# RexYing/gnn-model-explainer

Hardware: NVIDIA H100
Metric: explained-nodes/sec (100 mask-opt epochs each) (higher is better)
Workload: dtype f32

## Files before the change

### gnn-model-explainer_b200/csrc/api.cu

```cuda
#include <stdarg.h>
#include <stdio.h>
#include <stdlib.h>
#include <string.h>

#include <algorithm>
#include <cmath>
#include <iterator>
#include <memory>
#include <numeric>
#include <vector>

#include "host.cuh"

static thread_local char g_err[1024] = "";

void gx_set_error(const char* fmt, ...) {
  va_list ap;
  va_start(ap, fmt);
  vsnprintf(g_err, sizeof(g_err), fmt, ap);
  va_end(ap);
}

int check_node_list(const gx_handle* h, const char* who, const int32_t* nodes, int32_t count, int32_t n_hops, int min_hops) {
  if (n_hops < 1 || n_hops >= GX_MAX_LEVELS) { gx_set_error("%s: n_hops=%d outside [1,%d]", who, n_hops, GX_MAX_LEVELS - 1); return GX_ERR_INVALID; }
// ... 329 lines not shown
  cudaDeviceProp prop;
  GX_CUDA_CHECK(cudaGetDeviceProperties(&prop, device));
  if (prop.major != 9 || prop.minor != 0) {
    gx_set_error("gx_create: device %d is sm_%d%d; this library is built for sm_90a (H100) only", device, prop.major, prop.minor);
    return GX_ERR_CUDA;
  }
  auto h = std::make_unique<gx_handle>();
  h->device = device;
  h->num_sms = prop.multiProcessorCount;
  h->l2_bytes = prop.l2CacheSize;
  std::copy(std::begin(kNodeClasses), std::end(kNodeClasses), h->classes);
  if (const char* env = getenv("GNNX_CLASS_THREADS")) {
    int v[kNumClasses], k = 0;
    const char* p = env;
    while (*p && k < kNumClasses) { v[k++] = atoi(p); while (*p && *p != ',') ++p; if (*p == ',') ++p; }
    for (int c = 0; c < k; ++c) if (v[c] >= 32 && v[c] % 32 == 0 && (v[c] <= 256 || v[c] == 512)) h->classes[c].threads = v[c];
  }
  if (const char* env = getenv("GNNX_EXCLUSIVE_TOPK")) h->exclusive_topk = atoi(env);
  if (const char* env = getenv("GNNX_HOST_TIMING")) h->host_timing = env[0] == '1';
  if (const char* env = getenv("GNNX_FORCE_STREAM")) h->force_stream = atoi(env) != 0;
  if (const char* env = getenv("GNNX_GANG")) h->gang_override = atoi(env);
  if (const char* env = getenv("GNNX_CLUSTER_SIZE")) { const int v = atoi(env); if (v == 0 || v == 1 || v == 2 || v == 4) h->cluster_size = v; }
  if (const char* env = getenv("GNNX_CLUSTER_COST")) { const long long v = atoll(env); if (v > 0) h->cluster_cost = v; }
  if (const char* env = getenv("GNNX_IEEE_EDGE")) h->ieee_edge = atoi(env) != 0;
  if (const char* env = getenv("GNNX_NODE_GENERIC")) h->node_generic = atoi(env) != 0;
  for (int i = 0; i < kNumClasses; ++i) {
    GX_CUDA_CHECK(cudaStreamCreateWithFlags(&h->side[i], cudaStreamNonBlocking));
    GX_CUDA_CHECK(cudaEventCreate(&h->ev_join[i]));
    GX_CUDA_CHECK(cudaEventCreate(&h->ev_begin[i]));
  }
  GX_CUDA_CHECK(cudaEventCreateWithFlags(&h->ev_fork, cudaEventDisableTiming));
// ... 15 lines not shown
  if (!h) { gx_set_error("gx_set_stream: NULL handle"); return GX_ERR_INVALID; }
  h->stream = (cudaStream_t)cuda_stream;
  return GX_OK;
}

int gx_sync(gx_handle* h) {
  if (!h) { gx_set_error("gx_sync: NULL handle"); return GX_ERR_INVALID; }
  GX_CUDA_CHECK(cudaSetDevice(h->device));
  GX_CUDA_CHECK(cudaStreamSynchronize(h->stream));
  return GX_OK;
}

int64_t gx_launch_count(gx_handle* h) { return h ? h->launches : 0; }

int gx_debug_set_dump(gx_handle* h, float* dev_buf) { if (!h) return GX_ERR_INVALID; h->dbg = dev_buf; return GX_OK; }

int gx_debug_ieee_edge(gx_handle* h, int on) { if (!h) return GX_ERR_INVALID; h->ieee_edge = on != 0; return GX_OK; }

int gx_model_forward(gx_handle* h, gx_memspace space, float* pred) {
  if (!h || !pred) { gx_set_error("gx_model_forward: NULL argument"); return GX_ERR_INVALID; }
  if (!h->has_graph || !h->has_model) { gx_set_error("gx_model_forward: call gx_set_model and gx_set_graph_csr first"); return GX_ERR_INVALID; }
  if (h->g.d != h->m.d) { gx_set_error("gx_model_forward: graph feat_dim %d != model input_dim %d", h->g.d, h->m.d); return GX_ERR_INVALID; }
  GX_CUDA_CHECK(cudaSetDevice(h->device));
  const size_t np_ = (size_t)h->g.N * h->m.C;
  const size_t nh = (size_t)h->m.L * h->g.N * gx_var_row_stride(h->m.hid, h->m.emb);
  const size_t npw = h->m.att ? (size_t)h->g.N * gx_round_up(std::max(h->m.d, h->m.hid), 4) : 0;
  const size_t ne = h->head.k > 0 ? (size_t)h->g.N * (h->m.hid * (h->m.L - 1) + h->m.emb) : 0;
  GX_CUDA_CHECK(h->d_fwd.reserve((nh + np_ + npw + ne) * 4));
  float* H = h->d_fwd.as<float>();
  float* pd = space == GX_DEVICE ? pred : H + nh;
// ... 339 lines not shown
```

### gnn-model-explainer_b200/csrc/explain_common.cuh

```cuda
#pragma once
#include "gnnx_internal.cuh"

namespace {

#ifndef GX_SHORT_DEPTH
#define GX_SHORT_DEPTH 1
#endif
constexpr int kLongRow = 32;

__device__ __forceinline__ float warp_sum(float x) {
#pragma unroll
  for (int o = 16; o > 0; o >>= 1) x += __shfl_xor_sync(0xffffffffu, x, o);
  return x;
}
__device__ __forceinline__ float warp_max(float x) {
#pragma unroll
  for (int o = 16; o > 0; o >>= 1) x = fmaxf(x, __shfl_xor_sync(0xffffffffu, x, o));
  return x;
}
__device__ __forceinline__ float sigmoid_f(float x) { return 1.0f / (1.0f + expf(-x)); }
__device__ __forceinline__ float sigmoid_fast(float x, bool ieee) {
  return ieee ? 1.0f / (1.0f + expf(-x)) : __fdividef(1.0f, 1.0f + __expf(-x));
}
__device__ __forceinline__ float adam_delta_fast(float m, float v, float step, float bc2s, float bc2s_inv, float eps, bool ieee) {
// ... 260 lines not shown
```

### gnn-model-explainer_b200/csrc/explain_node.cu

```cuda
#include "explain_common.cuh"

namespace {

template <typename IdxT, int HID, int EMB, bool kWpShared, bool kTrace>
__device__ __forceinline__ void readout_phase(int lane, int C, int gt, const IdxT* irp, const IdxT* icol, const float* a,
                                              const float* Yh1, const float* Yh2, float* zs, const float* bs, const float* W3s,
                                              const float* Wpp, const float* bpp, float* logit, float* dE, float* dZ3,
                                              float* tr, float* trp) {
  constexpr int HS = HID, H4 = HID / 4, PD = 2 * HID + EMB;
  const int g = lane >> 3, q8 = lane & 7;
  float4 acc = make_float4(0.f, 0.f, 0.f, 0.f);
  {
    const int r0 = irp[0], r1 = irp[1];
    if (q8 < H4) acc = gather_row<IdxT, true, 4>(r0 + g, r1, 4, icol, a, Yh2, HS, q8);
  }
#pragma unroll
  for (int o = 8; o <= 16; o <<= 1) {
    acc.x += __shfl_xor_sync(0xffffffffu, acc.x, o); acc.y += __shfl_xor_sync(0xffffffffu, acc.y, o);
    acc.z += __shfl_xor_sync(0xffffffffu, acc.z, o); acc.w += __shfl_xor_sync(0xffffffffu, acc.w, o);
  }
  if (lane < H4) st4(zs + 4 * lane, acc);
  __syncwarp();
  const int le = lane < EMB ? lane : EMB - 1;
  const int lh = lane < HID ? lane : HID - 1;
// ... 110 lines not shown
    if (tid == 0 && crank == 0) peer.sti(&s_task, atomicAdd(A.counter, 1));
    phase_sync<CS>();
    const int qi = s_task;
    phase_sync<CS>();
    if (qi >= A.ntasks) break;
    const int task_id = A.order[qi];
    if (A.dbg != nullptr && tid == 0) {
      unsigned long long t_start_ns;
      asm volatile("mov.u64 %0, %%globaltimer;" : "=l"(t_start_ns));
      s_clk[7] = (long long)t_start_ns;
    }
    const GxTask* __restrict__ Tp = A.plan.tasks + task_id;
    const int n = Tp->n, n1 = Tp->n1, n2 = Tp->n2, e1 = Tp->e1, np = Tp->npairs_in;
    const int gt = hp.mode ? __ldg(A.g.pred_label + Tp->node) : Tp->gt_label;
    const int64_t node_off = Tp->node_off, rp_off = Tp->rp_off, edge_off = Tp->edge_off, pair_off = Tp->pair_off;
    if (tid == 0) sL = gx_make_layout(n, n1, n2, e1, d, HID, EMB, C, nwarps, (int)sizeof(IdxT), CS);
    __syncthreads();
    const int dp = sL.dp, D4 = dp / 4;
    const int32_t* __restrict__ lo2gid = A.plan.lo2gid + node_off;

    {
      float* const X = base + sL.X; float* const W1s = base + sL.W1s; float* const W2s = base + sL.W2s; float* const W3s = base + sL.W3s;
      float* const bs = base + sL.bs; float* const sF = base + sL.sF; float* const Fm = base + sL.F; float* const mF = base + sL.mF;
      float* const vF = base + sL.vF; float* const gFp = base + sL.gFp; float* const a = base + sL.a; float* const yv = base + sL.y;
      float2* const MM = reinterpret_cast<float2*>(A.pws + (int64_t)cid * A.pws_stride_words); float2* const mm = MM + np; float2* const vv = mm + np; float2* const SS = vv + np;
      uint2* const PX = reinterpret_cast<uint2*>(SS + np);
      IdxT* const icol = reinterpret_cast<IdxT*>(base + sL.icol); IdxT* const irp = reinterpret_cast<IdxT*>(base + sL.irp);
    for (int idx = tid; idx < n * dp; idx += nthreads) {
      const int i = idx / dp, f = idx - i * dp;
      X[idx] = f < d ? __ldg(A.g.feat + (int64_t)lo2gid[i] * d + f) : 0.f;
    }
    for (int idx = tid; idx < dp * HS; idx += nthreads) {
      const int f = idx / HS, c = idx - f * HS;
      W1s[idx] = f < d ? __ldg(m.W[0] + f * HID + c) : 0.f;
    }
    for (int idx = tid; idx < HID * HS; idx += nthreads) W2s[idx] = __ldg(m.W[1] + idx);
    {
      float* const W1t = base + sL.W1t; float* const W2t = base + sL.W2t;
      for (int idx = tid; idx < HID * dp; idx += nthreads) {
// ... 18 lines not shown
      sF[f] = hp.mode ? 1.0f : 0.5f;
      Fm[f] = 0.f; mF[f] = 0.f; vF[f] = 0.f;
      if (resume && A.x.feat_state_in != nullptr && f < d) {
        const float* fs = A.x.feat_state_in + (int64_t)task_id * 3 * d;
        Fm[f] = fs[f]; mF[f] = fs[d + f]; vF[f] = fs[2 * d + f];
        sF[f] = sigmoid_f(fs[f]);
      }
      if (hp.out_iter == 0 && !hp.mode && f < d) {
        if (A.out_feat != nullptr) A.out_feat[(int64_t)task_id * d + f] = sF[f];
        if (A.x.feat_state_out != nullptr) {
          float* fo = A.x.feat_state_out + (int64_t)task_id * 3 * d;
          fo[f] = Fm[f]; fo[d + f] = mF[f]; fo[2 * d + f] = vF[f];
        }
      }
    }
    for (int idx = tid; idx < cnwarps * dp; idx += nthreads) gFp[idx] = 0.f;
    const float m0_std = sqrtf(2.0f / (float)n);
    for (int p = tid; p < np; p += nthreads) {
      const int i = A.plan.pair_i[pair_off + p], j = A.plan.pair_j[pair_off + p];
      const int pij = A.plan.pair_pij[pair_off + p], pji = A.plan.pair_pji[pair_off + p];
      const int oij = A.plan.pair_oij[pair_off + p], oji = A.plan.pair_oji[pair_off + p];
      float Mi, Mj;
      if (hp.mode) {
        Mi = Mj = 0.f;
      } else if (hp.init == GX_INIT_PHILOX) {
        Mi = 1.0f + m0_std * philox_normal(hp.seed, (uint32_t)Tp->node, (uint32_t)oij);
        Mj = 1.0f + m0_std * philox_normal(hp.seed, (uint32_t)Tp->node, (uint32_t)oji);
      } else {
        Mi = __ldg(A.m0 + edge_off + oij);
        Mj = __ldg(A.m0 + edge_off + oji);
      }
// ... 204 lines not shown
            st4(dZ2 + j * HS + 4 * q, group_dense(zs + G.gbase * 4, H4, W2t, HS, q, make_float4(0.f, 0.f, 0.f, 0.f)));
          __syncwarp();
        }
      }
      __syncthreads();
      GX_MARK(3)
      {
        const IdxT* const irp = reinterpret_cast<const IdxT*>(base + sL.irp);
        const IdxT* const icol = reinterpret_cast<const IdxT*>(base + sL.icol);
        const float* const a = base + sL.a; const float* const dZ2 = base + sL.dZ2; const float* const dE = base + sL.dE;
        const float* const Yh1 = base + sL.Yh1; const float* const q1 = base + sL.q1; const float* const W1t = base + sL.W1t;
        const float* const U = base + sL.U; const float* const sF = base + sL.sF;
        const IdxT* const cnt1 = reinterpret_cast<const IdxT*>(base + sL.cnt1);
        const IdxT* const llistB = reinterpret_cast<const IdxT*>(base + sL.llistB);
        float* const dZ1s = base + sL.U;
        float* const gFp = base + sL.gFp; float* const zs = base + sL.zs + warp * 128;
        float4 gacc = make_float4(0.f, 0.f, 0.f, 0.f);
        const int ntask = nlongB1 + (n2 + epi - 1) / epi;
        for (int t = cwarp; t < ntask; t += cnwarps) {
          float4 dh;
          const int i = row_task_gather<IdxT, false, (NT >= 512 ? 1 : GX_SHORT_DEPTH)>(t, nlongB1, llistB, n2, G, H4, irp, icol, a, dZ2, HS, cnt1, zs, dh);
          const bool act = i >= 0;
          float4 yh = make_float4(0.f, 0.f, 0.f, 0.f), dy = yh;
          if (act && q < H4) {
            yh = ld4(Yh1 + i * HS + 4 * q);
            if (i == 0) { const float4 e4 = ld4(dE + 4 * q); dh.x += e4.x; dh.y += e4.y; dh.z += e4.z; dh.w += e4.w; }
            dy.x = yh.x > 0.f ? dh.x : 0.f; dy.y = yh.y > 0.f ? dh.y : 0.f;
            dy.z = yh.z > 0.f ? dh.z : 0.f; dy.w = yh.w > 0.f ? dh.w : 0.f;
          }
          const float sdot = group_sum<kGW>(yh.x * dy.x + yh.y * dy.y + yh.z * dy.z + yh.w * dy.w, G);
          if (act && q < H4) {
            const float rq = q1[i];
            st4(zs + lane * 4, make_float4((dy.x - yh.x * sdot) * rq, (dy.y - yh.y * sdot) * rq,
                                           (dy.z - yh.z * sdot) * rq, (dy.w - yh.w * sdot) * rq));
          }
          __syncwarp();
          if (act && q < D4) {
            const float4 o = group_dense(zs + G.gbase * 4, H4, W1t, dp, q, make_float4(0.f, 0.f, 0.f, 0.f));
            const float4 u = ld4(U + i * dp + 4 * q);
            const float4 s4 = ld4(sF + 4 * q);
            gacc.x = fmaf(o.x, u.x, gacc.x); gacc.y = fmaf(o.y, u.y, gacc.y);
            gacc.z = fmaf(o.z, u.z, gacc.z); gacc.w = fmaf(o.w, u.w, gacc.w);
            peer.st4(dZ1s + i * dp + 4 * q, make_float4(o.x * s4.x, o.y * s4.y, o.z * s4.z, o.w * s4.w));
          }
          __syncwarp();
        }
        st4(zs + lane * 4, gacc);
        __syncwarp();
        if (G.grp == 0 && q < D4) {
          float4 tsum = gacc;
          for (int g2 = 1; g2 < epi; ++g2) {
            const float4 o = ld4(zs + (g2 * G.GW + q) * 4);
            tsum.x += o.x; tsum.y += o.y; tsum.z += o.z; tsum.w += o.w;
          }
          peer.st4(gFp + cwarp * dp + 4 * q, tsum);
        }
        __syncwarp();
      }
      phase_sync<CS>();
      GX_MARK(4)
      if (A.dbg != nullptr && it == 1 && qi == 0 && crank == 0) {
        if (tid == 0) {
          A.dbg[0] = (float)sL.total_words; A.dbg[1] = (float)sL.X; A.dbg[2] = (float)sL.U; A.dbg[3] = (float)sL.Yh1;
          A.dbg[4] = (float)sL.q1; A.dbg[5] = (float)sL.Yh2; A.dbg[6] = (float)sL.q2; A.dbg[7] = (float)sL.dZ2;
          A.dbg[8] = (float)sL.U; A.dbg[9] = (float)sL.gFp; A.dbg[10] = (float)sL.dE; A.dbg[11] = (float)sL.dZ3;
          A.dbg[12] = (float)sL.logit; A.dbg[13] = (float)sL.a; A.dbg[14] = (float)dp; A.dbg[15] = (float)nwarps;
        }
        for (int w = tid; w < sL.total_words; w += nthreads) A.dbg[16 + w] = base[w];
      }
      {
        float* const gFp = base + sL.gFp;
        float* const sF = base + sL.sF;
        float* const Fm = base + sL.F; float* const mF = base + sL.mF; float* const vF = base + sL.vF;
        const float* const yv = base + sL.y;
        const float* const dZ1s = base + sL.U;
        float* const X = base + sL.X;
        float* const dZ2 = base + sL.dZ2;
        float* const Yh1 = base + sL.Yh1;
        float* const dZ3 = base + sL.dZ3;
        float* const Yh2 = base + sL.Yh2;
        float2* const MM = reinterpret_cast<float2*>(A.pws + (int64_t)cid * A.pws_stride_words); float2* const mm = MM + np; float2* const vv = mm + np; float2* const SS = vv + np;
        const uint2* const PX = reinterpret_cast<const uint2*>(SS + np);
        float* const a = base + sL.a;
        const int p0 = cwarp * 32 + lane, pstride = nthreads * CS;
        uint2 pxn = p0 < np ? PX[p0] : make_uint2(0u, 0u);
        const float2 tab = __ldg(hp.adam_tab + (it - 1));
        const float step = tab.x, bc2s = tab.y, bc2s_inv = 1.0f / tab.y;
        const bool last = (it == hp.out_iter);
        const float nn = (float)n * (float)n;
        const float ent_over_nn = hp.c_ent / nn;
        const float lap_over_nn = hp.c_lap / nn;
        const int fthreads = min(nthreads, gx_round_up(d, 32));
        for (int f = tid - (nthreads - fthreads); f >= 0 && f < d && !hp.mode; f += fthreads) {
          float gsum = 0.f;
          for (int w = 0; w < cnwarps; ++w) gsum += gFp[w * dp + f];
          const float s = sF[f];
          const float g = s * (1.f - s) * (gsum + hp.c_feat_size / (float)d);
          float mf = mF[f], vf = vF[f], Fv = Fm[f];
          mf = mf + (g - mf) * hp.one_minus_b1;
          vf = vf * hp.b2 + hp.one_minus_b2 * g * g;
          Fv = Fv - step * (mf / (sqrtf(vf) / bc2s + hp.eps));
          mF[f] = mf; vF[f] = vf; Fm[f] = Fv;
          const float sn = sigmoid_f(Fv);
          sF[f] = sn;
          if (last && crank == 0) {
            if (A.out_feat != nullptr) A.out_feat[(int64_t)task_id * d + f] = sn;
            if (A.x.feat_state_out != nullptr) {
              float* fo = A.x.feat_state_out + (int64_t)task_id * 3 * d;
              fo[f] = Fv; fo[d + f] = mf; fo[2 * d + f] = vf;
            }
// ... 201 lines not shown
template <typename IdxT, int HID, int EMB, int NT, int CS, bool kNarrow = false>
cudaError_t launch_one(const GxExplainLaunch& cfg, const ExplainArgs& args, cudaStream_t s) {
  if (args.x.trace != nullptr) return launch_one_t<IdxT, HID, EMB, NT, true, CS, kNarrow>(cfg, args, s);
  return launch_one_t<IdxT, HID, EMB, NT, false, CS, kNarrow>(cfg, args, s);
}

template <int HID, int EMB>
cudaError_t launch_dims(const GxExplainLaunch& cfg, const ExplainArgs& args, cudaStream_t s) {
  if (cfg.smem_bytes <= 0) return cudaErrorInvalidValue;
  if (cfg.cluster == 4) return launch_one<uint16_t, HID, EMB, 512, 4>(cfg, args, s);
  if (cfg.cluster == 2) return launch_one<uint16_t, HID, EMB, 512, 2>(cfg, args, s);
  if (cfg.cluster != 1) return cudaErrorInvalidValue;
  const bool narrow = HID == EMB && 4 * ((args.m.d + 3) / 4) <= HID && (args.hp.flags & GX_HP_NODE_GENERIC) == 0;
  if (cfg.threads <= 256)
    return narrow ? launch_one<uint16_t, HID, EMB, 256, 1, true>(cfg, args, s) : launch_one<uint16_t, HID, EMB, 256, 1>(cfg, args, s);
  return narrow ? launch_one<uint16_t, HID, EMB, 512, 1, true>(cfg, args, s) : launch_one<uint16_t, HID, EMB, 512, 1>(cfg, args, s);
}

}

int gx_explain_max_smem() { return 227 * 1024; }

cudaError_t gx_launch_outer_pairs(const GxHparamsDev& hp, const GxGraphDev& g, const GxPlanArrays& plan, int count,
                                  const float* m0, float* out_mask, const GxExtra& x, cudaStream_t s) {
  const int grid = count < GX_GRID_CAP ? count : GX_GRID_CAP;
  if (x.trace != nullptr) {
    const size_t smem = (size_t)(hp.iters > 0 ? hp.iters : 1) * 4 * sizeof(double);
    if (smem > 48 * 1024) return cudaErrorInvalidValue;
    outer_pairs_kernel<true><<<grid, 256, smem, s>>>(hp, g, plan, count, m0, out_mask, x);
  } else {
    const int slices = std::max(1, std::min(32, GX_GRID_CAP / grid));
    outer_pairs_kernel<false><<<dim3(grid, slices), 256, 0, s>>>(hp, g, plan, count, m0, out_mask, x);
  }
  return cudaGetLastError();
}

// ... 9 lines not shown
```

### gnn-model-explainer_b200/csrc/gnnx_internal.cuh

```cuda
#pragma once
#include <cuda_runtime.h>
#include <stdint.h>

#include "gnnx.h"

#define GX_MAX_LEVELS 8
#define GX_NONE16 0xFFFFu
#define GX_MAX_LAYERS 7
#define GX_MAX_GANG 160
#define GX_GRID_CAP (132 * 8)
#define GX_WP_SMEM_MAX 2048

struct GxTask {
  int32_t node;
  int32_t n;
  int32_t e_d;
  int32_t npairs;
  int32_t npairs_in;
  int32_t idx_new;
  int32_t gt_label;
  int32_t n1, n2;
  int32_t e1;
  int32_t status;
  int32_t n_norm;
// ... 82 lines not shown

#define GX_HP_IEEE_EDGE 1
#define GX_HP_NODE_GENERIC 2

struct GxExtra {
  float* trace;
  float* trace_pred;
  double* tr_outer;
  int32_t epochs;
  const float* adam_m_in; const float* adam_v_in; const float* feat_state_in;
  float* mask_param_out; float* adam_m_out; float* adam_v_out; float* feat_state_out;
};

__host__ __device__ inline int gx_round_up(int x, int m) { return (x + m - 1) / m * m; }

struct GxLayout {
  int X, U, Yh1, q1, Yh2, q2, dZ2, a, y, W1s, W1t, W2s, W2t, W3s, bs, sF, F, mF, vF, gFp, zs, dE, dZ3, logit, Wp;
  int icol, irp, llist, cnt1, llistB;
  int total_words;
  int dp;
};

__host__ __device__ inline GxLayout gx_make_layout(int n, int n1, int n2, int e1, int d,
                                                   int hid, int emb, int C, int nwarps,
                                                   int idx_bytes, int cs = 1) {
  GxLayout L;
  const int dp = gx_round_up(d, 4);
  L.dp = dp;
  int o = 0;
  auto takef = [&](int words) { int r = o; o += gx_round_up(words, 4); return r; };
  auto takei = [&](int elems) { int r = o; o += gx_round_up((elems * idx_bytes + 3) / 4, 4); return r; };
  L.X = takef(n * dp);
  L.U = takef(n2 * dp);
  L.Yh1 = takef(n2 * hid);
  L.q1 = takef(n2);
  L.Yh2 = takef(n1 * hid);
  L.q2 = takef(n1);
  L.dZ2 = takef(n1 * hid);
  L.a = takef(e1);
  L.y = takef(n);
  L.W1s = takef(dp * hid);
  L.W1t = takef(hid * dp);
  L.W2s = takef(hid * hid);
  L.W2t = takef(hid * hid);
  L.W3s = takef(hid * emb);
  L.bs = takef(2 * hid + emb);
  L.sF = takef(dp);
  L.F = takef(dp);
  L.mF = takef(dp);
  L.vF = takef(dp);
  L.gFp = takef(nwarps * cs * dp);
  L.zs = takef(nwarps * 128);
  L.dE = takef(2 * hid);
  L.dZ3 = takef(hid);
  L.logit = takef(C < 32 ? 32 : C);
  L.Wp = takef(C * (2 * hid + emb + 1) <= GX_WP_SMEM_MAX ? C * (2 * hid + emb + 1) : 0);
  L.icol = takei(e1);
  L.irp = takei(n2 + 1);
  L.llist = takei(n2);
  L.cnt1 = takei(n2);
  L.llistB = takei(n2);
  L.total_words = o;
  return L;
}

struct GxStreamLayout {
// ... 168 lines not shown
  int32_t grid;
  int32_t cluster = 1;
  int32_t gang = 1;
  unsigned long long* gang_bars = nullptr;
  int32_t* gang_mail = nullptr;
  float* gws;
  int64_t gws_stride_words;
  float* pws;
  int64_t pws_stride_words;
  float* dbg;
  GxExtra x;
};
cudaError_t gx_launch_explain(const GxExplainLaunch& cfg, const GxGraphDev& g, const GxModelDev& m,
                              const GxHparamsDev& hp, const GxPlanArrays& plan, const float* m0,
                              float* out_mask, float* out_feat, cudaStream_t s);
cudaError_t gx_launch_explain_stream(const GxExplainLaunch& cfg, const GxGraphDev& g, const GxModelDev& m,
                                     const GxHparamsDev& hp, const GxPlanArrays& plan, const float* m0,
                                     float* out_mask, float* out_feat, cudaStream_t s);
cudaError_t gx_launch_explain_gang(const GxExplainLaunch& cfg, const GxGraphDev& g, const GxModelDev& m,
                                   const GxHparamsDev& hp, const GxPlanArrays& plan, const float* m0,
                                   float* out_mask, float* out_feat, cudaStream_t s);
int gx_gang_smem_bytes(int d, int hid, int C);
cudaError_t gx_launch_model_forward(const GxGraphDev& g, const GxModelDev& m, const GxHeadDev& hd, float* H, float* pred, float* emb_out, float* P,
                                    cudaStream_t s);
constexpr int GX_STREAM_THREADS = 768;
int gx_explain_max_smem();
struct GxGraphBatchDev {
  int32_t num_graphs, max_nodes, d;
  const int32_t* rowptr;
  const int32_t* col;
// ... 53 lines not shown
```

### gnn-model-explainer_b200/csrc/host.cuh

```cuda
#pragma once
#include <stdio.h>

#include <algorithm>
#include <chrono>
#include <vector>

#include "gnnx_internal.cuh"

struct DevBuf {
  void* p = nullptr;
  size_t cap = 0;
  DevBuf() = default;
  DevBuf(const DevBuf&) = delete;
  DevBuf& operator=(const DevBuf&) = delete;
  DevBuf(DevBuf&& o) noexcept : p(o.p), cap(o.cap) { o.p = nullptr; o.cap = 0; }
  DevBuf& operator=(DevBuf&& o) noexcept { std::swap(p, o.p); std::swap(cap, o.cap); return *this; }
  ~DevBuf() { if (p) cudaFree(p); }
  cudaError_t reserve(size_t bytes) {
    if (bytes <= cap) return cudaSuccess;
    if (p) cudaFree(p);
    p = nullptr;
    cap = 0;
    size_t want = bytes + bytes / 4 + 256;
    cudaError_t e = cudaMalloc(&p, want);
    if (e == cudaSuccess) cap = want;
    return e;
  }
  template <typename T> T* as() const { return reinterpret_cast<T*>(p); }
};

struct LaunchClass {
  int cap_bytes;
  int threads;
  int ctas_per_sm;
};
constexpr LaunchClass kNodeClasses[] = {
    {13 * 1024, 128, 16}, {27 * 1024, 256, 8}, {55 * 1024, 256, 4},
    {112 * 1024, 512, 2}, {226 * 1024, 512, 1}, {0, 512, 1}, {226 * 1024, 512, 1}};
constexpr int kNumClasses = sizeof(kNodeClasses) / sizeof(kNodeClasses[0]);
constexpr int kStreamClass = 5;
constexpr int kClusterClass = 6;
constexpr int kOneClass = 4, kTwoClass = 3;

inline double now_us() { return std::chrono::duration<double, std::micro>(std::chrono::steady_clock::now().time_since_epoch()).count(); }

struct AdamKey { float lr, b1, b2, decay_rate; int32_t opt, sched, decay_step, restart, iters, start; };

struct gx_handle {
  int device = 0;
  int num_sms = 132;
  int64_t l2_bytes = (int64_t)50 << 20;
  cudaStream_t stream = nullptr;
  cudaStream_t side[kNumClasses] = {};
  cudaEvent_t ev_fork = nullptr;
  cudaEvent_t ev_t0 = nullptr, ev_t1 = nullptr;
  bool timed = false;
  float* dbg = nullptr;
  LaunchClass classes[kNumClasses];
  int exclusive_topk = 30;
  bool host_timing = false;
  bool ieee_edge = false;
  bool node_generic = false;
  int gang_override = 0;
  int cluster_size = 1;
  int64_t cluster_cost = 0;
  int plan_cluster = 1;
  bool force_stream = false;
  cudaEvent_t ev_join[kNumClasses] = {}, ev_begin[kNumClasses] = {};
  bool class_used[kNumClasses] = {};
  int64_t launches = 0;

  bool has_graph = false;
  GxGraphDev g{};
  DevBuf g_rowptr, g_col, g_feat, g_label, g_pred;
// ... 151 lines not shown
```

### gnn-model-explainer_b200/csrc/node_mode.cu

```cuda
#include <string.h>

#include <algorithm>
#include <vector>

#include "host.cuh"

namespace {

int ensure_slot_ws(gx_handle* h) {
  const int64_t N = h->g.N;
  const int W = (int)((N + 31) / 32);
  int slots = h->num_sms * 8;
  const size_t per_slot = (size_t)W * 4 + (size_t)(W + 1) * 4 + (size_t)N + (size_t)(N + 1) * 4 * 2 + (size_t)N * 4 * 2 + 64;
  const size_t budget = (size_t)4 << 30;
  while (slots > 1 && per_slot * slots > budget) slots /= 2;
  if (h->ws.slots == slots && h->ws.W == W && h->ws_buf.p) return GX_OK;
  auto al = [](size_t x) { return (x + 15) / 16 * 16; };
  size_t o = 0;
  const size_t o_bm = o; o += al((size_t)slots * W * 4);
  const size_t o_wp = o; o += al((size_t)slots * (W + 1) * 4);
  const size_t o_q = o; o += al((size_t)slots * (N + 1) * 4);
  const size_t o_loc = o; o += al((size_t)slots * N * 4);
  const size_t o_cof = o; o += al((size_t)slots * N * 4);
  const size_t o_pb = o; o += al((size_t)slots * (N + 1) * 4);
// ... 5 lines not shown
  h->ws.q = (int32_t*)(b + o_q);
  h->ws.loc = (int32_t*)(b + o_loc);
  h->ws.cof = (int32_t*)(b + o_cof);
  h->ws.pbase = (int32_t*)(b + o_pb);
  h->ws.dist = (uint8_t*)(b + o_dist);
  h->ws.W = W;
  h->ws.slots = slots;
  GX_CUDA_CHECK(cudaMemsetAsync(h->ws.bm, 0, (size_t)slots * W * 4, h->stream));
  return GX_OK;
}

int task_smem_class(const gx_handle* h, const GxTask& T, int* bytes_out) {
  const GxModelDev& m = h->m;
  const bool small_idx = !h->force_stream && T.n < 65535 && T.e1 < 65535;
  for (int c = 0; small_idx && c < kStreamClass; ++c) {
    const int nwarps = h->classes[c].threads / 32;
    const GxLayout L = gx_make_layout(T.n, T.n1, T.n2, T.e1, m.d, m.hid, m.emb, m.C, nwarps, 2);
    const int64_t bytes = (int64_t)L.total_words * 4;
    if (bytes <= h->classes[c].cap_bytes) {
      *bytes_out = (int)bytes;
      return c;
    }
  }
  *bytes_out = 0;
  return kStreamClass;
}

enum class NodeKernel { smem, cluster, gang, stream1, variant };

}

// ... 115 lines not shown
  h->plan.pair_pji = pb + 3 * tp; h->plan.pair_oij = pb + 4 * tp; h->plan.pair_oji = pb + 5 * tp;
  const double t2 = h->host_timing ? now_us() : 0.0;
  GX_CUDA_CHECK(gx_launch_khop_fill(h->g, count, n_hops, h->ws, h->plan, h->stream));
  h->launches += 1;
  const LaunchClass& cluster_cls = h->classes[kClusterClass];
  for (int c = 0; c < kNumClasses; ++c) h->class_order[c].clear();
  auto cost = [&](int32_t t) { const GxTask& T = h->tasks[t]; return (int64_t)T.e1 * (h->m.d + 2 * h->m.hid) + (int64_t)T.n2 * 600 + (int64_t)T.npairs * 60; };
  const int g_cluster_size = h->cluster_size > 1 ? h->cluster_size : 1;
  const int64_t g_cluster_cost = h->cluster_cost;
  h->plan_cluster = g_cluster_size;
  for (int t = 0; t < count; ++t) {
    GxTask& T = h->tasks[t];
    int bytes = 0;
    int cls = h->m.variant ? kStreamClass : task_smem_class(h, T, &bytes);
    if (cls < kStreamClass && g_cluster_size > 1 && cost(t) > g_cluster_cost) {
      const GxLayout L = gx_make_layout(T.n, T.n1, T.n2, T.e1, h->m.d, h->m.hid, h->m.emb, h->m.C, cluster_cls.threads / 32, 2, g_cluster_size);
      if ((int64_t)L.total_words * 4 <= cluster_cls.cap_bytes) { cls = kClusterClass; bytes = L.total_words * 4; }
    }
    T.smem_bytes = bytes;
    h->class_order[cls].push_back(t);
  }
  if (h->cluster_size == 0 && !h->m.variant && !h->force_stream && h->class_order[kStreamClass].empty()) {
    double demand = 0;
    for (int c = 0; c < kStreamClass; ++c) demand += (double)h->class_order[c].size() / h->classes[c].ctas_per_sm;
    const int spare = h->num_sms - (int)(demand + 0.999);
    std::vector<int32_t> cand;
    for (int c : {kTwoClass, kOneClass}) for (int32_t t : h->class_order[c]) cand.push_back(t);
    std::stable_sort(cand.begin(), cand.end(), [&](int32_t x, int32_t y) { return cost(x) > cost(y); });
    auto lat = [&](int32_t t) { return 6e-6 * (double)cost(t); };
    int best_cs = 1, best_k = 0;
    if (!cand.empty() && spare >= 2) {
      double best = lat(cand[0]);
      for (int cs : {2, 4}) {
        const double ovh = cs == 2 ? 0.55 : 0.8;
        int k = 0;
        while (k < (int)cand.size() && (k + 1) * cs <= spare && lat(cand[k]) / cs + ovh < lat(cand[k])) {
          const GxTask& T = h->tasks[cand[k]];
          const GxLayout L = gx_make_layout(T.n, T.n1, T.n2, T.e1, h->m.d, h->m.hid, h->m.emb, h->m.C, cluster_cls.threads / 32, 2, cs);
          if ((int64_t)L.total_words * 4 > cluster_cls.cap_bytes) break;
          ++k;
        }
        if (k == 0) continue;
        const double span = std::max(lat(cand[0]) / cs + ovh, k < (int)cand.size() ? lat(cand[k]) : 0.0);
        if (span < best * 0.95) { best = span; best_cs = cs; best_k = k; }
      }
    }
    if (best_cs > 1) {
      h->plan_cluster = best_cs;
      for (int i = 0; i < best_k; ++i) {
        const int32_t t = cand[i];
        GxTask& T = h->tasks[t];
        const GxLayout L = gx_make_layout(T.n, T.n1, T.n2, T.e1, h->m.d, h->m.hid, h->m.emb, h->m.C, cluster_cls.threads / 32, 2, best_cs);
        T.smem_bytes = L.total_words * 4;
        for (int c : {kTwoClass, kOneClass}) {
          auto& v = h->class_order[c];
          v.erase(std::remove(v.begin(), v.end(), t), v.end());
        }
        h->class_order[kClusterClass].push_back(t);
      }
    }
  }
  std::vector<int32_t> order_all;
  for (int c = 0; c < kNumClasses; ++c) {
    auto& v = h->class_order[c];
    std::stable_sort(v.begin(), v.end(), [&](int32_t x, int32_t y) { return cost(x) > cost(y); });
  }
  {
// ... 91 lines not shown
      const LaunchClass& K = h->classes[c];
      const int nt = (int)h->class_order[c].size();
      int need = 0;
      for (int32_t t : h->class_order[c]) need = std::max(need, h->tasks[t].smem_bytes);
      cfg[c].threads = K.threads;
      cfg[c].dbg = h->dbg;
      cfg[c].x = D.x;
      if (c == kClusterClass) {
        kernel[c] = NodeKernel::cluster;
        cfg[c].cluster = h->plan_cluster;
        cfg[c].grid = std::min<int>(nt, h->num_sms / h->plan_cluster) * h->plan_cluster;
        cfg[c].smem_bytes = std::max(need, K.cap_bytes - 2048);
        slabs[c] = cfg[c].grid / h->plan_cluster;
      } else if (K.cap_bytes > 0) {
        kernel[c] = NodeKernel::smem;
        cfg[c].grid = std::min<int>(nt, h->num_sms * K.ctas_per_sm);
        cfg[c].smem_bytes = c == kOneClass ? std::max(need, K.cap_bytes - 2048) : std::max(need, 1024);
        slabs[c] = cfg[c].grid;
      } else if (nt > 0) {
        int max_slabs = h->num_sms, gang = 0;
        if (!h->m.variant && h->gang_override >= 0 && h->m.d <= 128 && gx_gang_smem_bytes(h->m.d, h->m.hid, h->m.C) <= gx_explain_max_smem()) {
          int64_t ws = 1;
          for (int32_t t : h->class_order[c]) ws = std::max<int64_t>(ws, (int64_t)h->tasks[t].e_d * 8 + (int64_t)h->tasks[t].n * 240);
          const int64_t l2_budget = h->l2_bytes * 5 / 8;
          int ngangs = (int)std::max<int64_t>(1, std::min<int64_t>(std::min(nt, h->num_sms), l2_budget / ws));
          gang = std::max(1, std::min(h->num_sms / ngangs, GX_MAX_GANG));
          if (h->gang_override > 0) gang = std::min(std::min(h->gang_override, h->num_sms), GX_MAX_GANG);
          max_slabs = std::max(1, std::min(ngangs, h->num_sms / gang));
        }
        kernel[c] = h->m.variant ? NodeKernel::variant : gang > 0 ? NodeKernel::gang : NodeKernel::stream1;
// ... 74 lines not shown
```

### gnn-model-explainer_b200/gnnx/_abi.py

```python
import ctypes as C
import os

_HERE = os.path.dirname(os.path.abspath(__file__))
LIB_PATH = os.environ.get("GNNX_LIB_PATH") or os.path.join(_HERE, "lib", "libgnnx.so")

GX_OK = 0
GX_ERR_UNSUPPORTED = -3
GX_HOST, GX_DEVICE = 0, 1
GX_INIT_M0, GX_INIT_PHILOX, GX_INIT_STATE = 0, 1, 2
GX_VERSION = 211
GX_TRACE_COLS = 8
TR_LOSS_EDGES, TR_PRED, TR_SIZE, TR_ENT, TR_LAP, TR_FEAT, TR_DENSITY, TR_PGT = range(8)
GX_MODEL_BN = 1
GX_MODEL_ATT = 2
GX_MAX_HEAD_LAYERS = 4

EXPORTS = [
    "gx_default_hparams", "gx_last_error", "gx_version", "gx_create", "gx_destroy", "gx_set_stream",
    "gx_sync", "gx_set_model", "gx_set_graph_csr", "gx_neighborhood_rows", "gx_plan_nodes",
    "gx_plan_fetch", "gx_explain_nodes", "gx_densify", "gx_launch_count", "gx_last_explain_ms",
    "gx_set_graph_batch_csr", "gx_plan_graphs", "gx_explain_graphs", "gx_grad_nodes", "gx_grad_graphs",
    "gx_explain_nodes_ex", "gx_explain_graphs_ex", "gx_offedge_regularisers", "gx_offedge_regularisers_graphs",
    "gx_debug_force_stream", "gx_debug_ieee_edge", "gx_debug_set_dump", "gx_debug_set_gang", "gx_debug_set_cluster", "gx_denoise_topk",
    "gx_model_forward", "gx_comm_unique_id", "gx_comm_init", "gx_comm_destroy", "gx_count_nodes", "gx_allgather_masks", "gx_unshard_masks",
    "gx_plan_class_counts", "gx_last_class_ms", "gx_explain_nodes_unconstrained", "gx_explain_graphs_unconstrained",
    "gx_set_model_att", "gx_set_model_head", "gx_count_graphs", "gx_densify_graphs", "gx_denoise_topk_edges",
]


class GxModelDims(C.Structure):
    _fields_ = [("input_dim", C.c_int32), ("hidden_dim", C.c_int32), ("embed_dim", C.c_int32),
                ("num_classes", C.c_int32), ("num_layers", C.c_int32), ("flags", C.c_int32)]


class GxHparams(C.Structure):
    _fields_ = [("num_epochs", C.c_int32), ("lr", C.c_float), ("beta1", C.c_float), ("beta2", C.c_float),
                ("eps", C.c_float), ("coef_size", C.c_float), ("coef_feat_size", C.c_float),
                ("coef_ent", C.c_float), ("coef_lap", C.c_float), ("mask_act", C.c_int32),
# ... 61 lines not shown
    L.gx_grad_nodes.argtypes = [vp, C.c_int, f32p]
    L.gx_grad_graphs.argtypes = [vp, C.c_int, i32p, f32p]
    L.gx_denoise_topk.argtypes = [vp, C.c_int, f32p, C.c_int32, C.c_int32, f32p, i32p, i32p, f32p]
    L.gx_denoise_topk_edges.argtypes = [vp, C.c_int, f32p, C.c_int32, C.c_int32, f32p, i32p, i32p, f32p]
    L.gx_comm_unique_id.argtypes = [C.c_char_p]
    L.gx_comm_init.argtypes = [vp, C.c_int32, C.c_int32, C.c_char_p]
    L.gx_comm_destroy.argtypes = [vp]
    L.gx_count_nodes.argtypes = [vp, i32p, C.c_int32, C.c_int32, i32p, i32p]
    L.gx_allgather_masks.argtypes = [vp, f32p, C.c_int64, C.c_int64, f32p]
    L.gx_unshard_masks.argtypes = [vp, f32p, C.c_int32, i64p, i64p, i32p, f32p]
    L.gx_count_graphs.argtypes = [vp, i32p, C.c_int32, i32p, i32p]
    L.gx_densify_graphs.argtypes = [vp, C.c_int, i32p, C.c_int32, f32p, vp]
    L.gx_debug_force_stream.argtypes = [vp, C.c_int]
    L.gx_debug_ieee_edge.argtypes = [vp, C.c_int]
    L.gx_debug_set_dump.argtypes = [vp, vp]
    L.gx_model_forward.argtypes = [vp, C.c_int, f32p]
    L.gx_debug_set_gang.argtypes = [vp, C.c_int]
    L.gx_debug_set_cluster.argtypes = [vp, C.c_int, C.c_int64]
    L.gx_launch_count.argtypes = [vp]
    L.gx_plan_class_counts.argtypes = [vp, i32p, i32p, i32p]
    L.gx_last_class_ms.argtypes = [vp, f32p, f32p]
    L.gx_launch_count.restype = C.c_int64
    L.gx_last_explain_ms.argtypes = [vp, C.POINTER(C.c_float)]
    for name in EXPORTS:
        getattr(L, name)
    if L.gx_version() != GX_VERSION:
        raise ImportError("libgnnx.so is version %d, this binding expects %d -- rebuild (python __graft_entry__.py)" % (L.gx_version(), GX_VERSION))
    _lib = L
    return L

# ... 5 lines not shown
```

### include/gnnx.h

```cpp
#ifndef GNNX_H_
#define GNNX_H_

#include <stdint.h>

#ifdef __cplusplus
extern "C" {
#endif

#define GX_VERSION 211

typedef struct gx_handle gx_handle;

typedef enum gx_status {
  GX_OK = 0,
  GX_ERR_INVALID = -1,
  GX_ERR_CUDA = -2,
  GX_ERR_UNSUPPORTED = -3,
  GX_ERR_NODE = -4,
  GX_ERR_NOMEM = -5
} gx_status;

typedef enum gx_memspace { GX_HOST = 0, GX_DEVICE = 1 } gx_memspace;

typedef struct gx_model_dims {
// ... 139 lines not shown
int gx_count_graphs(gx_handle* h, const int32_t* graph_ids, int32_t count, int32_t* n_out, int32_t* e_out);
int gx_densify_graphs(gx_handle* h, gx_memspace space, const int32_t* graph_ids, int32_t count, const float* values, double* out);

int gx_model_forward(gx_handle* h, gx_memspace space, float* pred);

int64_t gx_launch_count(gx_handle* h);
int gx_plan_class_counts(gx_handle* h, int32_t counts[7], int32_t smem_bytes[7], int32_t* cluster_size);
int gx_last_class_ms(gx_handle* h, float begin_ms[7], float end_ms[7]);
int gx_last_explain_ms(gx_handle* h, float* ms);

int gx_debug_set_gang(gx_handle* h, int ctas_per_task);
int gx_debug_set_cluster(gx_handle* h, int cluster_size, int64_t min_cost);
int gx_debug_force_stream(gx_handle* h, int on);
int gx_debug_ieee_edge(gx_handle* h, int on);
int gx_debug_set_dump(gx_handle* h, float* dev_buf);

#ifdef __cplusplus
}
#endif
#endif
```

Measured before the change: 212,500.

## Store per-task feature-grad partials and compute CTA residency from occupancy API

Replaces the per-warp feature-gradient accumulator (sized by warps times cluster size) with a per-task partial buffer sized by a task-count bound. The final reduction now sums over tasks instead of over warps, which removes the zero-initialisation pass and makes the layout independent of warp count. CTAs-per-SM for each launch class is now queried from the CUDA occupancy API rather than hardcoded, and the defaults for the small classes drop from 16/8 to 8/4. The change also adds an optional 1024-thread variant and lowers the exclusive top-k default. Risks include larger shared memory for tasks with many B1 rows, and lower residency if the occupancy query is conservative.

```diff
diff --git a/gnn-model-explainer_b200/csrc/api.cu b/gnn-model-explainer_b200/csrc/api.cu
--- a/gnn-model-explainer_b200/csrc/api.cu
+++ b/gnn-model-explainer_b200/csrc/api.cu
@@ -367,7 +367,14 @@
     int v[kNumClasses], k = 0;
     const char* p = env;
     while (*p && k < kNumClasses) { v[k++] = atoi(p); while (*p && *p != ',') ++p; if (*p == ',') ++p; }
-    for (int c = 0; c < k; ++c) if (v[c] >= 32 && v[c] % 32 == 0 && (v[c] <= 256 || v[c] == 512)) h->classes[c].threads = v[c];
+    for (int c = 0; c < k; ++c)
+      if (v[c] >= 32 && v[c] % 32 == 0 && (v[c] <= 256 || v[c] == 512 || (v[c] == 1024 && c != kClusterClass))) h->classes[c].threads = v[c];
+  }
+  for (int c = 0; c < kNumClasses; ++c) {
+    if (h->classes[c].cap_bytes == 0) continue;
+    const int n = gx_node_ctas_per_sm(h->classes[c].threads, h->classes[c].cap_bytes);
+    if (n < 1) { gx_set_error("gx_create: launch class %d (%d threads, %d bytes) fits no SM", c, h->classes[c].threads, h->classes[c].cap_bytes); return GX_ERR_CUDA; }
+    h->classes[c].ctas_per_sm = n;
   }
   if (const char* env = getenv("GNNX_EXCLUSIVE_TOPK")) h->exclusive_topk = atoi(env);
   if (const char* env = getenv("GNNX_HOST_TIMING")) h->host_timing = env[0] == '1';
@@ -413,6 +420,15 @@
 int64_t gx_launch_count(gx_handle* h) { return h ? h->launches : 0; }
 
 int gx_debug_set_dump(gx_handle* h, float* dev_buf) { if (!h) return GX_ERR_INVALID; h->dbg = dev_buf; return GX_OK; }
+
+int gx_debug_class_residency(gx_handle* h, int32_t threads[7], int32_t ctas_per_sm[7]) {
+  if (!h) return GX_ERR_INVALID;
+  for (int c = 0; c < kNumClasses; ++c) {
+    if (threads) threads[c] = h->classes[c].threads;
+    if (ctas_per_sm) ctas_per_sm[c] = h->classes[c].ctas_per_sm;
+  }
+  return GX_OK;
+}
 
 int gx_debug_ieee_edge(gx_handle* h, int on) { if (!h) return GX_ERR_INVALID; h->ieee_edge = on != 0; return GX_OK; }
 
diff --git a/gnn-model-explainer_b200/csrc/explain_common.cuh b/gnn-model-explainer_b200/csrc/explain_common.cuh
--- a/gnn-model-explainer_b200/csrc/explain_common.cuh
+++ b/gnn-model-explainer_b200/csrc/explain_common.cuh
@@ -6,7 +6,6 @@
 #ifndef GX_SHORT_DEPTH
 #define GX_SHORT_DEPTH 1
 #endif
-constexpr int kLongRow = 32;
 
 __device__ __forceinline__ float warp_sum(float x) {
 #pragma unroll
diff --git a/gnn-model-explainer_b200/csrc/explain_node.cu b/gnn-model-explainer_b200/csrc/explain_node.cu
--- a/gnn-model-explainer_b200/csrc/explain_node.cu
+++ b/gnn-model-explainer_b200/csrc/explain_node.cu
@@ -148,7 +148,7 @@
     const int n = Tp->n, n1 = Tp->n1, n2 = Tp->n2, e1 = Tp->e1, np = Tp->npairs_in;
     const int gt = hp.mode ? __ldg(A.g.pred_label + Tp->node) : Tp->gt_label;
     const int64_t node_off = Tp->node_off, rp_off = Tp->rp_off, edge_off = Tp->edge_off, pair_off = Tp->pair_off;
-    if (tid == 0) sL = gx_make_layout(n, n1, n2, e1, d, HID, EMB, C, nwarps, (int)sizeof(IdxT), CS);
+    if (tid == 0) sL = gx_make_layout(n, n1, n2, e1, d, HID, EMB, C, nwarps, (int)sizeof(IdxT));
     __syncthreads();
     const int dp = sL.dp, D4 = dp / 4;
     const int32_t* __restrict__ lo2gid = A.plan.lo2gid + node_off;
@@ -156,7 +156,7 @@
     {
       float* const X = base + sL.X; float* const W1s = base + sL.W1s; float* const W2s = base + sL.W2s; float* const W3s = base + sL.W3s;
       float* const bs = base + sL.bs; float* const sF = base + sL.sF; float* const Fm = base + sL.F; float* const mF = base + sL.mF;
-      float* const vF = base + sL.vF; float* const gFp = base + sL.gFp; float* const a = base + sL.a; float* const yv = base + sL.y;
+      float* const vF = base + sL.vF; float* const a = base + sL.a; float* const yv = base + sL.y;
       float2* const MM = reinterpret_cast<float2*>(A.pws + (int64_t)cid * A.pws_stride_words); float2* const mm = MM + np; float2* const vv = mm + np; float2* const SS = vv + np;
       uint2* const PX = reinterpret_cast<uint2*>(SS + np);
       IdxT* const icol = reinterpret_cast<IdxT*>(base + sL.icol); IdxT* const irp = reinterpret_cast<IdxT*>(base + sL.irp);
@@ -205,7 +205,6 @@
         }
       }
     }
-    for (int idx = tid; idx < cnwarps * dp; idx += nthreads) gFp[idx] = 0.f;
     const float m0_std = sqrtf(2.0f / (float)n);
     for (int p = tid; p < np; p += nthreads) {
       const int i = A.plan.pair_i[pair_off + p], j = A.plan.pair_j[pair_off + p];
@@ -440,8 +439,7 @@
         const IdxT* const cnt1 = reinterpret_cast<const IdxT*>(base + sL.cnt1);
         const IdxT* const llistB = reinterpret_cast<const IdxT*>(base + sL.llistB);
         float* const dZ1s = base + sL.U;
-        float* const gFp = base + sL.gFp; float* const zs = base + sL.zs + warp * 128;
-        float4 gacc = make_float4(0.f, 0.f, 0.f, 0.f);
+        float* const gFt = base + sL.gFt; float* const zs = base + sL.zs + warp * 128;
         const int ntask = nlongB1 + (n2 + epi - 1) / epi;
         for (int t = cwarp; t < ntask; t += cnwarps) {
           float4 dh;
@@ -461,27 +459,26 @@
                                            (dy.z - yh.z * sdot) * rq, (dy.w - yh.w * sdot) * rq));
           }
           __syncwarp();
+          float4 ou = make_float4(0.f, 0.f, 0.f, 0.f);
           if (act && q < D4) {
             const float4 o = group_dense(zs + G.gbase * 4, H4, W1t, dp, q, make_float4(0.f, 0.f, 0.f, 0.f));
             const float4 u = ld4(U + i * dp + 4 * q);
             const float4 s4 = ld4(sF + 4 * q);
-            gacc.x = fmaf(o.x, u.x, gacc.x); gacc.y = fmaf(o.y, u.y, gacc.y);
-            gacc.z = fmaf(o.z, u.z, gacc.z); gacc.w = fmaf(o.w, u.w, gacc.w);
+            ou = make_float4(o.x * u.x, o.y * u.y, o.z * u.z, o.w * u.w);
             peer.st4(dZ1s + i * dp + 4 * q, make_float4(o.x * s4.x, o.y * s4.y, o.z * s4.z, o.w * s4.w));
           }
           __syncwarp();
-        }
-        st4(zs + lane * 4, gacc);
-        __syncwarp();
-        if (G.grp == 0 && q < D4) {
-          float4 tsum = gacc;
-          for (int g2 = 1; g2 < epi; ++g2) {
-            const float4 o = ld4(zs + (g2 * G.GW + q) * 4);
-            tsum.x += o.x; tsum.y += o.y; tsum.z += o.z; tsum.w += o.w;
-          }
-          peer.st4(gFp + cwarp * dp + 4 * q, tsum);
-        }
-        __syncwarp();
+          st4(zs + lane * 4, ou);
+          __syncwarp();
+          if (G.grp == 0 && q < D4) {
+            for (int g2 = 1; g2 < epi; ++g2) {
+              const float4 o = ld4(zs + (g2 * G.GW + q) * 4);
+              ou.x += o.x; ou.y += o.y; ou.z += o.z; ou.w += o.w;
+            }
+            peer.st4(gFt + t * dp + 4 * q, ou);
+          }
+          __syncwarp();
+        }
       }
       phase_sync<CS>();
       GX_MARK(4)
@@ -489,13 +486,14 @@
         if (tid == 0) {
           A.dbg[0] = (float)sL.total_words; A.dbg[1] = (float)sL.X; A.dbg[2] = (float)sL.U; A.dbg[3] = (float)sL.Yh1;
           A.dbg[4] = (float)sL.q1; A.dbg[5] = (float)sL.Yh2; A.dbg[6] = (float)sL.q2; A.dbg[7] = (float)sL.dZ2;
-          A.dbg[8] = (float)sL.U; A.dbg[9] = (float)sL.gFp; A.dbg[10] = (float)sL.dE; A.dbg[11] = (float)sL.dZ3;
-          A.dbg[12] = (float)sL.logit; A.dbg[13] = (float)sL.a; A.dbg[14] = (float)dp; A.dbg[15] = (float)nwarps;
+          A.dbg[8] = (float)sL.U; A.dbg[9] = (float)sL.gFt; A.dbg[10] = (float)sL.dE; A.dbg[11] = (float)sL.dZ3;
+          A.dbg[12] = (float)sL.logit; A.dbg[13] = (float)sL.a; A.dbg[14] = (float)dp; A.dbg[15] = (float)(nlongB1 + (n2 + epi - 1) / epi);
         }
         for (int w = tid; w < sL.total_words; w += nthreads) A.dbg[16 + w] = base[w];
       }
       {
-        float* const gFp = base + sL.gFp;
+        const float* const gFt = base + sL.gFt;
+        const int ntaskB1 = nlongB1 + (n2 + epi - 1) / epi;
         float* const sF = base + sL.sF;
         float* const Fm = base + sL.F; float* const mF = base + sL.mF; float* const vF = base + sL.vF;
         const float* const yv = base + sL.y;
@@ -519,7 +517,8 @@
         const int fthreads = min(nthreads, gx_round_up(d, 32));
         for (int f = tid - (nthreads - fthreads); f >= 0 && f < d && !hp.mode; f += fthreads) {
           float gsum = 0.f;
-          for (int w = 0; w < cnwarps; ++w) gsum += gFp[w * dp + f];
+#pragma unroll 4
+          for (int t = 0; t < ntaskB1; ++t) gsum += gFt[t * dp + f];
           const float s = sF[f];
           const float g = s * (1.f - s) * (gsum + hp.c_feat_size / (float)d);
           float mf = mF[f], vf = vF[f], Fv = Fm[f];
@@ -751,12 +750,33 @@
   const bool narrow = HID == EMB && 4 * ((args.m.d + 3) / 4) <= HID && (args.hp.flags & GX_HP_NODE_GENERIC) == 0;
   if (cfg.threads <= 256)
     return narrow ? launch_one<uint16_t, HID, EMB, 256, 1, true>(cfg, args, s) : launch_one<uint16_t, HID, EMB, 256, 1>(cfg, args, s);
-  return narrow ? launch_one<uint16_t, HID, EMB, 512, 1, true>(cfg, args, s) : launch_one<uint16_t, HID, EMB, 512, 1>(cfg, args, s);
+  if (cfg.threads <= 512)
+    return narrow ? launch_one<uint16_t, HID, EMB, 512, 1, true>(cfg, args, s) : launch_one<uint16_t, HID, EMB, 512, 1>(cfg, args, s);
+  if (cfg.threads != 1024 || args.x.trace != nullptr) return cudaErrorInvalidValue;
+  return narrow ? launch_one_t<uint16_t, HID, EMB, 1024, false, 1, true>(cfg, args, s) : launch_one_t<uint16_t, HID, EMB, 1024, false, 1, false>(cfg, args, s);
+}
+
+template <int NT>
+int ctas_per_sm(int threads, int smem_bytes) {
+  auto kern = explain_node_kernel<uint16_t, 20, 20, NT, false, 1, true>;
+  int n = 0;
+  if (cudaFuncSetAttribute(kern, cudaFuncAttributeMaxDynamicSharedMemorySize, smem_bytes) != cudaSuccess ||
+      cudaFuncSetAttribute(kern, cudaFuncAttributePreferredSharedMemoryCarveout, cudaSharedmemCarveoutMaxShared) != cudaSuccess ||
+      cudaOccupancyMaxActiveBlocksPerMultiprocessor(&n, kern, threads, (size_t)smem_bytes) != cudaSuccess)
+    return 0;
+  return n;
 }
 
 }
 
 int gx_explain_max_smem() { return 227 * 1024; }
+
+int gx_node_ctas_per_sm(int threads, int smem_bytes) {
+  if (threads < 32 || threads % 32 != 0) return 0;
+  if (threads <= 256) return ctas_per_sm<256>(threads, smem_bytes);
+  if (threads <= 512) return ctas_per_sm<512>(threads, smem_bytes);
+  return threads == 1024 ? ctas_per_sm<1024>(threads, smem_bytes) : 0;
+}
 
 cudaError_t gx_launch_outer_pairs(const GxHparamsDev& hp, const GxGraphDev& g, const GxPlanArrays& plan, int count,
                                   const float* m0, float* out_mask, const GxExtra& x, cudaStream_t s) {
diff --git a/gnn-model-explainer_b200/csrc/gnnx_internal.cuh b/gnn-model-explainer_b200/csrc/gnnx_internal.cuh
--- a/gnn-model-explainer_b200/csrc/gnnx_internal.cuh
+++ b/gnn-model-explainer_b200/csrc/gnnx_internal.cuh
@@ -120,8 +120,19 @@
 
 __host__ __device__ inline int gx_round_up(int x, int m) { return (x + m - 1) / m * m; }
 
+constexpr int kLongRow = 32;
+
+__host__ __device__ inline int gx_b1_task_bound(int n1, int n2, int e1, int d, int hid, int emb) {
+  int gw = (d + 3) / 4;
+  gw = gw > hid / 4 ? gw : hid / 4;
+  gw = gw > emb / 4 ? gw : emb / 4;
+  const int epi = gw <= 32 ? 32 / gw : 1;
+  const int nlong = n1 > kLongRow ? (n2 < e1 / (kLongRow + 1) ? n2 : e1 / (kLongRow + 1)) : 0;
+  return (n2 + epi - 1) / epi + nlong;
+}
+
 struct GxLayout {
-  int X, U, Yh1, q1, Yh2, q2, dZ2, a, y, W1s, W1t, W2s, W2t, W3s, bs, sF, F, mF, vF, gFp, zs, dE, dZ3, logit, Wp;
+  int X, U, Yh1, q1, Yh2, q2, dZ2, a, y, W1s, W1t, W2s, W2t, W3s, bs, sF, F, mF, vF, gFt, zs, dE, dZ3, logit, Wp;
   int icol, irp, llist, cnt1, llistB;
   int total_words;
   int dp;
@@ -129,7 +140,7 @@
 
 __host__ __device__ inline GxLayout gx_make_layout(int n, int n1, int n2, int e1, int d,
                                                    int hid, int emb, int C, int nwarps,
-                                                   int idx_bytes, int cs = 1) {
+                                                   int idx_bytes) {
   GxLayout L;
   const int dp = gx_round_up(d, 4);
   L.dp = dp;
@@ -155,7 +166,7 @@
   L.F = takef(dp);
   L.mF = takef(dp);
   L.vF = takef(dp);
-  L.gFp = takef(nwarps * cs * dp);
+  L.gFt = takef(gx_b1_task_bound(n1, n2, e1, d, hid, emb) * dp);
   L.zs = takef(nwarps * 128);
   L.dE = takef(2 * hid);
   L.dZ3 = takef(hid);
@@ -354,6 +365,7 @@
 cudaError_t gx_launch_explain(const GxExplainLaunch& cfg, const GxGraphDev& g, const GxModelDev& m,
                               const GxHparamsDev& hp, const GxPlanArrays& plan, const float* m0,
                               float* out_mask, float* out_feat, cudaStream_t s);
+int gx_node_ctas_per_sm(int threads, int smem_bytes);
 cudaError_t gx_launch_explain_stream(const GxExplainLaunch& cfg, const GxGraphDev& g, const GxModelDev& m,
                                      const GxHparamsDev& hp, const GxPlanArrays& plan, const float* m0,
                                      float* out_mask, float* out_feat, cudaStream_t s);
diff --git a/gnn-model-explainer_b200/csrc/host.cuh b/gnn-model-explainer_b200/csrc/host.cuh
--- a/gnn-model-explainer_b200/csrc/host.cuh
+++ b/gnn-model-explainer_b200/csrc/host.cuh
@@ -35,7 +35,7 @@
   int ctas_per_sm;
 };
 constexpr LaunchClass kNodeClasses[] = {
-    {13 * 1024, 128, 16}, {27 * 1024, 256, 8}, {55 * 1024, 256, 4},
+    {13 * 1024, 128, 8}, {27 * 1024, 256, 4}, {55 * 1024, 256, 4},
     {112 * 1024, 512, 2}, {226 * 1024, 512, 1}, {0, 512, 1}, {226 * 1024, 512, 1}};
 constexpr int kNumClasses = sizeof(kNodeClasses) / sizeof(kNodeClasses[0]);
 constexpr int kStreamClass = 5;
@@ -57,7 +57,7 @@
   bool timed = false;
   float* dbg = nullptr;
   LaunchClass classes[kNumClasses];
-  int exclusive_topk = 30;
+  int exclusive_topk = 22;
   bool host_timing = false;
   bool ieee_edge = false;
   bool node_generic = false;
diff --git a/gnn-model-explainer_b200/csrc/node_mode.cu b/gnn-model-explainer_b200/csrc/node_mode.cu
--- a/gnn-model-explainer_b200/csrc/node_mode.cu
+++ b/gnn-model-explainer_b200/csrc/node_mode.cu
@@ -43,7 +43,7 @@
   const GxModelDev& m = h->m;
   const bool small_idx = !h->force_stream && T.n < 65535 && T.e1 < 65535;
   for (int c = 0; small_idx && c < kStreamClass; ++c) {
-    const int nwarps = h->classes[c].threads / 32;
+    const int nwarps = std::min(h->classes[c].threads, 512) / 32;
     const GxLayout L = gx_make_layout(T.n, T.n1, T.n2, T.e1, m.d, m.hid, m.emb, m.C, nwarps, 2);
     const int64_t bytes = (int64_t)L.total_words * 4;
     if (bytes <= h->classes[c].cap_bytes) {
@@ -189,7 +189,7 @@
     int bytes = 0;
     int cls = h->m.variant ? kStreamClass : task_smem_class(h, T, &bytes);
     if (cls < kStreamClass && g_cluster_size > 1 && cost(t) > g_cluster_cost) {
-      const GxLayout L = gx_make_layout(T.n, T.n1, T.n2, T.e1, h->m.d, h->m.hid, h->m.emb, h->m.C, cluster_cls.threads / 32, 2, g_cluster_size);
+      const GxLayout L = gx_make_layout(T.n, T.n1, T.n2, T.e1, h->m.d, h->m.hid, h->m.emb, h->m.C, cluster_cls.threads / 32, 2);
       if ((int64_t)L.total_words * 4 <= cluster_cls.cap_bytes) { cls = kClusterClass; bytes = L.total_words * 4; }
     }
     T.smem_bytes = bytes;
@@ -211,7 +211,7 @@
         int k = 0;
         while (k < (int)cand.size() && (k + 1) * cs <= spare && lat(cand[k]) / cs + ovh < lat(cand[k])) {
           const GxTask& T = h->tasks[cand[k]];
-          const GxLayout L = gx_make_layout(T.n, T.n1, T.n2, T.e1, h->m.d, h->m.hid, h->m.emb, h->m.C, cluster_cls.threads / 32, 2, cs);
+          const GxLayout L = gx_make_layout(T.n, T.n1, T.n2, T.e1, h->m.d, h->m.hid, h->m.emb, h->m.C, cluster_cls.threads / 32, 2);
           if ((int64_t)L.total_words * 4 > cluster_cls.cap_bytes) break;
           ++k;
         }
@@ -225,7 +225,7 @@
       for (int i = 0; i < best_k; ++i) {
         const int32_t t = cand[i];
         GxTask& T = h->tasks[t];
-        const GxLayout L = gx_make_layout(T.n, T.n1, T.n2, T.e1, h->m.d, h->m.hid, h->m.emb, h->m.C, cluster_cls.threads / 32, 2, best_cs);
+        const GxLayout L = gx_make_layout(T.n, T.n1, T.n2, T.e1, h->m.d, h->m.hid, h->m.emb, h->m.C, cluster_cls.threads / 32, 2);
         T.smem_bytes = L.total_words * 4;
         for (int c : {kTwoClass, kOneClass}) {
           auto& v = h->class_order[c];
@@ -347,6 +347,16 @@
         slabs[c] = cfg[c].grid / h->plan_cluster;
       } else if (K.cap_bytes > 0) {
         kernel[c] = NodeKernel::smem;
+        if (K.threads > 512) {
+          bool fits = D.x.trace == nullptr;
+          for (int32_t t : h->class_order[c]) {
+            const GxTask& T = h->tasks[t];
+            const int64_t bytes = (int64_t)gx_make_layout(T.n, T.n1, T.n2, T.e1, h->m.d, h->m.hid, h->m.emb, h->m.C, K.threads / 32, 2).total_words * 4;
+            fits = fits && bytes <= K.cap_bytes;
+            need = std::max<int>(need, (int)std::min<int64_t>(bytes, K.cap_bytes));
+          }
+          cfg[c].threads = fits ? K.threads : 512;
+        }
         cfg[c].grid = std::min<int>(nt, h->num_sms * K.ctas_per_sm);
         cfg[c].smem_bytes = c == kOneClass ? std::max(need, K.cap_bytes - 2048) : std::max(need, 1024);
         slabs[c] = cfg[c].grid;
diff --git a/gnn-model-explainer_b200/gnnx/_abi.py b/gnn-model-explainer_b200/gnnx/_abi.py
--- a/gnn-model-explainer_b200/gnnx/_abi.py
+++ b/gnn-model-explainer_b200/gnnx/_abi.py
@@ -21,7 +21,7 @@
     "gx_plan_fetch", "gx_explain_nodes", "gx_densify", "gx_launch_count", "gx_last_explain_ms",
     "gx_set_graph_batch_csr", "gx_plan_graphs", "gx_explain_graphs", "gx_grad_nodes", "gx_grad_graphs",
     "gx_explain_nodes_ex", "gx_explain_graphs_ex", "gx_offedge_regularisers", "gx_offedge_regularisers_graphs",
-    "gx_debug_force_stream", "gx_debug_ieee_edge", "gx_debug_set_dump", "gx_debug_set_gang", "gx_debug_set_cluster", "gx_denoise_topk",
+    "gx_debug_force_stream", "gx_debug_ieee_edge", "gx_debug_set_dump", "gx_debug_class_residency", "gx_debug_set_gang", "gx_debug_set_cluster", "gx_denoise_topk",
     "gx_model_forward", "gx_comm_unique_id", "gx_comm_init", "gx_comm_destroy", "gx_count_nodes", "gx_allgather_masks", "gx_unshard_masks",
     "gx_plan_class_counts", "gx_last_class_ms", "gx_explain_nodes_unconstrained", "gx_explain_graphs_unconstrained",
     "gx_set_model_att", "gx_set_model_head", "gx_count_graphs", "gx_densify_graphs", "gx_denoise_topk_edges",
@@ -113,6 +113,7 @@
     L.gx_debug_force_stream.argtypes = [vp, C.c_int]
     L.gx_debug_ieee_edge.argtypes = [vp, C.c_int]
     L.gx_debug_set_dump.argtypes = [vp, vp]
+    L.gx_debug_class_residency.argtypes = [vp, vp, vp]
     L.gx_model_forward.argtypes = [vp, C.c_int, f32p]
     L.gx_debug_set_gang.argtypes = [vp, C.c_int]
     L.gx_debug_set_cluster.argtypes = [vp, C.c_int, C.c_int64]
diff --git a/include/gnnx.h b/include/gnnx.h
--- a/include/gnnx.h
+++ b/include/gnnx.h
@@ -177,6 +177,7 @@
 int gx_debug_force_stream(gx_handle* h, int on);
 int gx_debug_ieee_edge(gx_handle* h, int on);
 int gx_debug_set_dump(gx_handle* h, float* dev_buf);
+int gx_debug_class_residency(gx_handle* h, int32_t threads[7], int32_t ctas_per_sm[7]);
 
 #ifdef __cplusplus
 }
```

New measurement: 216,600, median of 6. 1.9% higher.
